# adamgreig/basebandboard

Measured on AMD Instinct MI355X. Metric: awgn_clt_gsamples_per_s, higher is better.
Workload: dtype u32 bit-sliced GF(2) / int8 out

## Files before the change

### basebandboard_amd/csrc/awgn_kernels.hip

```cpp
#include "bbb_common.hpp"
#include "bitslice_util.hpp"
#include "awgn_launch.hpp"
#include "stage_common.hpp"

#include <cstdlib>
#include <mutex>
#include <type_traits>
#include "gen/lutopt256_gen.inc"

namespace bbb {


template <int W32, typename TabPtr>
__device__ __forceinline__ void nibble_matvec_part(TabPtr tab, int nlo, int nhi, const uint32_t (&x)[W32],
                                                   uint32_t (&y)[W32]) {
    constexpr int C = (W32 % 4 == 0) ? 4 : (W32 % 2 == 0 ? 2 : 1);
    constexpr int NC = W32 / C;
    typedef uint32_t chunk_t __attribute__((ext_vector_type(C)));
#pragma unroll
    for (int w = 0; w < W32; w++) {
        uint32_t xw = x[w];
        asm volatile("" : "+v"(xw));
#pragma unroll
        for (int q = 0; q < 8; q += 2) {
// ... 457 lines not shown
        }
        auto load_windows = [&](const unsigned ihalf, uint32_t (&win)[16]) {
#pragma unroll
            for (unsigned e = 0; e < 16; e++) {
                const unsigned j = 8 * (e >> 2) + 4 * ihalf + (e & 3);
                const unsigned long long g = gen_index(wave, lane, j);
                win[e] = 0;
                if (g < G && tx.use_bits) {
                    const uint32_t off = (uint32_t)g * L + r * 16u;
                    const uint32_t rel = (off >> 3) + tx.rel_base;
                    const uint32_t byte = min(rel >> 3, tx.last_word * 4u - 4u);
                    typedef uint32_t __attribute__((aligned(1))) u32_unaligned;
                    win[e] = *reinterpret_cast<const u32_unaligned *>(reinterpret_cast<const char *>(tx.bits) + byte);
                }
            }
        };
        asm volatile("" ::: "memory");
        auto load_z = [&](const unsigned i, uint32_t (&zz)[16]) {
#pragma unroll
            for (int w = 0; w < 4; w++)
#pragma unroll
                for (int t = 0; t < 4; t++) zz[4 * w + t] = Z[((4 * w + t) * 8 + i) * 64 + lane];
        };
        auto round_end = [&](auto full_c, const unsigned i, const uint32_t (&w4)[4], const uint32_t (&zz)[16]) {
            constexpr bool FULL = decltype(full_c)::value;
            uint32_t o[4][4];
#pragma unroll
            for (int w = 0; w < 4; w++) {
                uint32_t z[4] = {zz[4 * w], zz[4 * w + 1], zz[4 * w + 2], zz[4 * w + 3]};
                transpose4x4_bytes(z);
#pragma unroll
                for (int q = 0; q < 4; q++) o[w][q] = z[q];
            }
            u32x4 RA[TX ? 4 : 1], RB[TX ? 4 : 1], RC[TX ? 4 : 1];
            if (TX) {
#pragma unroll
                for (unsigned q = 0; q < 4; q++) {
                    const uint32_t gq = (uint32_t)gen_index(wave, lane, 8 * q + i);
                    const uint32_t rel_q = ((gq * L + r * 16u) >> 3) + tx.rel_base;
                    const uint32_t Q4 = ((w4[q] >> (rel_q & 7u)) & 0x3ffu) << 4;
                    RA[q] = *reinterpret_cast<const u32x4 *>(reinterpret_cast<const char *>(TT) + (Q4 & 0xff0u));
                    RB[q] = *reinterpret_cast<const u32x4 *>(reinterpret_cast<const char *>(TT) + ((Q4 >> 1) & 0xff0u));
                    RC[q] = *reinterpret_cast<const u32x4 *>(reinterpret_cast<const char *>(TT) + ((Q4 >> 2) & 0xff0u));
                }
            }
#pragma unroll
            for (unsigned q = 0; q < 4; q++) {
                const unsigned long long g = gen_index(wave, lane, 8 * q + i);
                const unsigned long long off = g * L + (unsigned long long)r * 16;
                if (!FULL && !(g < G && off < nsamples)) continue;
                if (!TX) {
                    int8_t *dst = (int8_t *)dst_;
                    const u32x4 v = {o[0][q], o[1][q], o[2][q], o[3][q]};
                    if (FULL || off + 16 <= nsamples) {
                        *reinterpret_cast<u32x4 *>(dst + off) = v;
                    } else {
                        const unsigned n = (unsigned)(nsamples - off);
                        for (unsigned e = 0; e < n; e++) dst[off + e] = (int8_t)((o[e >> 2][q] >> (8 * (e & 3))) & 0xff);
                    }
                } else {
                    int16_t *dst = (int16_t *)dst_;
                    const u32x4 A = RA[q], B = RB[q], C = RC[q];
                    const u16x2 nv16 = {(uint16_t)(tx.noise_var * 16), (uint16_t)(tx.noise_var * 16)};
                    uint32_t x[8];
#pragma unroll
                    for (int w = 0; w < 4; w++) {
                        const uint32_t u = o[w][q] ^ 0x80808080u;
                        const uint32_t u01 = __builtin_amdgcn_perm(0u, u, 0x0c010c00u);
                        const uint32_t u23 = __builtin_amdgcn_perm(0u, u, 0x0c030c02u);
                        const int d0 = (2 * w) & 3, d1 = (2 * w + 1) & 3;
                        const uint32_t s01 = w < 2 ? bfi_uniform(selmask[d0], A[d0], B[d0]) : bfi_uniform(selmask[d0], B[d0], C[d0]);
                        const uint32_t s23 = w < 2 ? bfi_uniform(selmask[d1], A[d1], B[d1]) : bfi_uniform(selmask[d1], B[d1], C[d1]);
                        const u16x2 m01 = __builtin_bit_cast(u16x2, u01) * nv16 + __builtin_bit_cast(u16x2, s01);
                        const u16x2 m23 = __builtin_bit_cast(u16x2, u23) * nv16 + __builtin_bit_cast(u16x2, s23);
                        x[2 * w] = __builtin_bit_cast(uint32_t, __builtin_bit_cast(i16x2, m01) >> 4);
                        x[2 * w + 1] = __builtin_bit_cast(uint32_t, __builtin_bit_cast(i16x2, m23) >> 4);
                    }
                    if (FULL || off + 16 <= nsamples) {
                        const u32x4 lo = {x[0], x[1], x[2], x[3]}, hi = {x[4], x[5], x[6], x[7]};
                        reinterpret_cast<u32x4 *>(dst + off)[0] = lo;
                        reinterpret_cast<u32x4 *>(dst + off)[1] = hi;
                    } else {
                        const unsigned n = (unsigned)(nsamples - off);
                        for (unsigned e = 0; e < n; e++) dst[off + e] = (int16_t)((x[e >> 1] >> (16 * (e & 1))) & 0xffff);
                    }
                }
            }
        };
        auto all_iterations = [&](auto full_c) {
            if (TX) {
#pragma unroll 1
                for (unsigned ihalf = 0; ihalf < 2; ihalf++) {
                    uint32_t win[16];
                    load_windows(ihalf, win);
                    uint32_t zc[16], zn[16];
                    load_z(4 * ihalf, zn);
#pragma unroll
                    for (unsigned ii = 0; ii < 4; ii++) {
#pragma unroll
                        for (int e = 0; e < 16; e++) zc[e] = zn[e];
                        if (ii < 3) load_z(4 * ihalf + ii + 1, zn);
                        const uint32_t w4[4] = {win[ii], win[4 + ii], win[8 + ii], win[12 + ii]};
                        round_end(full_c, 4 * ihalf + ii, w4, zc);
                    }
                }
            } else {
                const uint32_t none[4] = {0, 0, 0, 0};
                uint32_t zc[16], zn[16];
                load_z(0, zn);
#pragma unroll 1
                for (unsigned i = 0; i < 8; i++) {
#pragma unroll
                    for (int e = 0; e < 16; e++) zc[e] = zn[e];
                    load_z((i + 1) & 7, zn);
                    round_end(full_c, i, none, zc);
                }
            }
        };
        if (wave_full) all_iterations(std::true_type{});
        else all_iterations(std::false_type{});
    }
}

template <bool SMALL>
__global__ void __launch_bounds__(64) __attribute__((amdgpu_waves_per_eu(1, 1)))
awgn256_planes_kernel(const uint32_t *__restrict planes, u32x4 *__restrict stage, unsigned L, unsigned nlanes
) {
    const unsigned lane = threadIdx.x;
    const unsigned long long wave = blockIdx.x;
    const unsigned long long LG = wave * 64 + lane;
    __builtin_amdgcn_s_setprio(3);
    uint32_t a[256], b[256], pa[256], pb[256], cnt[8];
    if constexpr (SMALL) {
#ifdef BBB_SMALL_THROTTLE
        asm volatile("" ::: BBB_SMALL_THROTTLE);
#endif
        const uint32_t voff = (uint32_t)LG * 4u;
#define BBB_PLANE(p) (*reinterpret_cast<const uint32_t *>(reinterpret_cast<const char *>(planes + (size_t)(p) * nlanes) + (unsigned long long)voff))
#define BBB_PARK(p) { const uint32_t v_ = BBB_PLANE(p); BBB_ACC_WRITE(pa[p], v_); }
        LUTOPT256_FOR_PARKED_HI(BBB_PARK)
#undef BBB_PARK
#pragma unroll
        for (int p = 0; p < 256; p++)
            if (!lutopt256_hi_is_parked(p)) a[p] = BBB_PLANE(p);
#undef BBB_PLANE
    } else {
#pragma unroll
        for (int p = 0; p < 256; p++) b[p] = planes[(size_t)p * nlanes + LG];
        lutopt256_advance(b, a);
#define BBB_PARK(p) BBB_ACC_WRITE(pa[p], a[p]);
        LUTOPT256_FOR_PARKED_HI(BBB_PARK)
#undef BBB_PARK
    }
    u32x4 *out = stage_row(stage, wave, L, lane);
#pragma unroll 1
    for (unsigned t = 0; t < L; t += 2) {
        lutopt256_step_parked_hi(a, pa, b, pb, cnt);
        {
        __builtin_nontemporal_store((u32x4){cnt[0], cnt[1], cnt[2], cnt[3]}, out);
        __builtin_nontemporal_store((u32x4){cnt[4], cnt[5], cnt[6], cnt[7]}, out + kStageHalfVecs);
        }
        lutopt256_step_parked_hi(b, pb, a, pa, cnt);
        {
        __builtin_nontemporal_store((u32x4){cnt[0], cnt[1], cnt[2], cnt[3]}, out + kStageStepVecs);
        __builtin_nontemporal_store((u32x4){cnt[4], cnt[5], cnt[6], cnt[7]}, out + kStageStepVecs + kStageHalfVecs);
        }
        out += 2 * kStageStepVecs;
    }
}

int awgn256_planes_launch(const uint32_t *d_planes, void *stage, unsigned L, unsigned nlanes, hipStream_t st, bool small_footprint) {
    if (L & 1) return fail(BBB_EINVAL, "segment length must be even");
    if (small_footprint)
        hipLaunchKernelGGL(awgn256_planes_kernel<true>, dim3(nlanes / 64), dim3(64), 0, st, d_planes, (u32x4 *)stage, L, nlanes);
    else
        hipLaunchKernelGGL(awgn256_planes_kernel<false>, dim3(nlanes / 64), dim3(64), 0, st, d_planes, (u32x4 *)stage, L, nlanes);
    BBB_HIP(hipGetLastError());
    return BBB_OK;
}

constexpr unsigned kUnplaneRaw = kStageUnitBytes, kUnplaneLds = 3 * kStageUnitBytes, kUnplaneLdsTx = kUnplaneLds + 32 * 1024 + 2 * 2048;

template <bool TXM, bool NOWRAP = false>
__global__ void __launch_bounds__(256, 7)
unplane_kernel(const u32x4 *__restrict stage, char *__restrict dst, unsigned long long win_lo, unsigned long long nbytes_, unsigned L,
               unsigned long long G, StageGeom ge, TxFuse tx) {
    extern __shared__ __attribute__((aligned(16))) uint32_t lds[];
    typedef __attribute__((address_space(3))) void *lds_void_ptr;
    const unsigned tid = threadIdx.x, lane = tid & 63;
    const unsigned wv = (unsigned)__builtin_amdgcn_readfirstlane((int)(tid >> 6));
    if (blockIdx.x * ge.per_block >= ge.nunits) return;
    char *const dstw = dst - win_lo;
    const unsigned long long nbytes = win_lo + nbytes_;
    const unsigned l8 = tid & 7, qs = tid >> 3;
    const unsigned wr0 = l8 * 32 + ((((qs >> 2) ^ (2 * ((l8 >> 1) & 3))) << 2) | (qs & 3));
    const unsigned lq = (tid >> 3) & 7, c2 = tid & 7;
    const unsigned rd0 = (wv * 8 + lq) * 32 + ((c2 ^ (2 * ((lq >> 1) & 3))) << 2);
    uint32_t *const tile = lds + 2 * (kUnplaneRaw / 4);
    uint32_t *const T10 = lds + kUnplaneLds / 4;
    uint32_t *const winb = lds + kUnplaneLds / 4 + 8192;
    if (TXM) {
        uint16_t *const TT = reinterpret_cast<uint16_t *>(tile);
        for (int e = (int)tid; e < 256 * 8; e += 256) {
            const int q = e >> 3, j = e & 7, ph = (int)((tx.c0 + (unsigned)j) & 7u);
            int sum = 0;
#pragma unroll
            for (int idx = 0; idx < 8; idx++) {
                const int c = tx.coeffs[8 * idx + ph];
                sum += ((q >> (7 - idx)) & 1) ? c : -c;
            }
            const int shaped = tx.bit_en ? ((int)((unsigned)sum << 20) >> 20) : 0;
            TT[e] = (uint16_t)((unsigned)((shaped - 128 * tx.noise_var) * (NOWRAP ? 1 : 16)) & 0xffffu);
        }
        __syncthreads();
        for (unsigned p = tid; p < 1024 * 8; p += 256) {
            const unsigned q10 = p >> 3, e = 2 * (p & 7);
            const uint32_t lo = TT[(((q10 >> ((tx.c0 + e) >> 3)) & 0xffu) << 3) + (e & 7)];
            const uint32_t hi = TT[(((q10 >> ((tx.c0 + e + 1) >> 3)) & 0xffu) << 3) + ((e + 1) & 7)];
            T10[p] = lo | (hi << 16);
        }
        __syncthreads();
    }
    auto dma_unit = [&](const StagePos &p, unsigned buf) {
        stage_dma_unit(stage, ge, p, L, lds + buf * (kUnplaneRaw / 4), wv, lane);
        if (TXM) {
            const unsigned step0 = p.rg * kStageUnitSteps;
            const unsigned long long wabs = (unsigned long long)ge.w_lo + p.w;
            const long long so = (long long)((wabs * 2048 + p.q8 * 8) * (unsigned long long)L + step0) - (long long)win_lo;
#pragma unroll
            for (unsigned i = 0; i < 2; i++) {
                const unsigned e = (wv * 2 + i) * 64 + lane, row = e >> 1;
                const long long pu = so + (long long)((unsigned long long)((row >> 3) * 64 + (row & 7)) * L);
                uint32_t word = 0;
                if (pu > -128 && pu < (long long)nbytes_) word = (((uint32_t)(pu >> 3) + tx.rel_base) >> 5) + (e & 1);
                word = word < tx.last_word ? word : tx.last_word;
                __builtin_amdgcn_global_load_lds((const void *)(tx.bits + word), (lds_void_ptr)(uintptr_t)(winb + buf * 512 + (wv * 2 + i) * 64), 4, 0, 0);
            }
        }
    };
    auto wait_vm = [](unsigned n) {
        switch (n) {
#define BBB_W(N) case N: asm volatile("s_waitcnt vmcnt(" #N ")" ::: "memory"); break;
            BBB_W(8) BBB_W(10) BBB_W(16) BBB_W(26)
#undef BBB_W
        default: asm volatile("s_waitcnt vmcnt(0)" ::: "memory"); break;
        }
    };
    constexpr unsigned NDMA = TXM ? 10 : 8, NST = TXM ? 16 : 8;
    StagePos cur;
    const unsigned n_it = stage_block_units(ge, blockIdx.x, &cur);
    StagePos nxt = cur;
    stage_advance(nxt, ge);
    unsigned buf = 0;
    bool fast1 = false;
    dma_unit(cur, 0);
    for (unsigned it = 0; it < n_it; it++, buf ^= 1) {
        const unsigned q8 = cur.q8, step0 = cur.rg * 128;
        const unsigned long long w = (unsigned long long)ge.w_lo + cur.w;
        const bool more1 = it + 1 < n_it;
        if (more1) dma_unit(nxt, buf ^ 1);
        wait_vm((more1 ? NDMA : 0u) + (fast1 ? NST : 0u));
        __builtin_amdgcn_s_barrier();
        {
            uint32_t Z[4][8];
            stage_unpack<TXM>(lds + buf * (kUnplaneRaw / 4), tid, Z);
#pragma unroll
            for (unsigned s = 0; s < 4; s++) planes8_to_bytes(Z[s]);
#pragma unroll
            for (unsigned i = 0; i < 8; i++) {
                uint32_t z[4] = {Z[0][i], Z[1][i], Z[2][i], Z[3][i]};
                transpose4x4_bytes(z);
#pragma unroll
                for (unsigned q = 0; q < 4; q++) tile[wr0 + (8 * q + i) * 256] = z[q];
            }
        }
        asm volatile("s_waitcnt lgkmcnt(0)" ::: "memory");
        __builtin_amdgcn_s_barrier();
        const unsigned inseg = step0 + c2 * 16;
        const unsigned long long g0 = (w * 32 + wv) * 64 + q8 * 8 + lq;
        unsigned long long off = g0 * (unsigned long long)L + inseg;
        const unsigned long long goff = 256ull * L;
        const bool lane_fast = inseg < L && g0 + 7 * 256 < G && off >= win_lo && off + 7 * goff + 16 <= nbytes;
        const bool wave_fast = __all(lane_fast);
        fast1 = wave_fast;
        if (!TXM && inseg < L) {
            if (wave_fast) {
#pragma unroll
                for (unsigned k = 0; k < 8; k++) {
                    const u32x4 v = *reinterpret_cast<const u32x4 *>(&tile[rd0 + k * 1024]);
                    *reinterpret_cast<u32x4 *>(dstw + off) = v;
                    off += goff;
                }
            } else {
                for (unsigned k = 0; k < 8; k++, off += goff) {
                    if (g0 + 256ull * k >= G || off >= nbytes) break;
                    if (off < win_lo) continue;
                    const u32x4 v = *reinterpret_cast<const u32x4 *>(&tile[rd0 + k * 1024]);
                    if (off + 16 <= nbytes) {
                        *reinterpret_cast<u32x4 *>(dstw + off) = v;
                    } else {
                        const unsigned n = (unsigned)(nbytes - off);
                        for (unsigned e = 0; e < n; e++) dstw[off + e] = (char)((v[e >> 2] >> (8 * (e & 3))) & 0xff);
                    }
                }
            }
        }
        if (TXM && inseg < L) {
            int16_t *const dst16 = reinterpret_cast<int16_t *>(dst);
            const u16x2 nv16 = {(uint16_t)(tx.noise_var * (NOWRAP ? 1 : 16)), (uint16_t)(tx.noise_var * (NOWRAP ? 1 : 16))};
            const uint32_t idx_mask = tx.use_bits ? 0x7fe0u : 0u;
            const uint32_t sh = ((((uint32_t)((long long)(off - win_lo) >> 3)) + tx.rel_base - 2u * c2) & 31u) + 2u * c2;
            const uint32_t *const wb0 = winb + buf * 512 + (wv * 8 + lq) * 2;
            auto piece = [&](auto full_c, unsigned k, unsigned long long o) {
                constexpr bool FULL = decltype(full_c)::value;
                typedef uint32_t u32x2 __attribute__((ext_vector_type(2)));
                const u32x2 ww = *reinterpret_cast<const u32x2 *>(wb0 + k * 64);
                const u32x4 v = *reinterpret_cast<const u32x4 *>(&tile[rd0 + k * 1024]);
                const uint32_t wk = (uint32_t)((((unsigned long long)ww[1] << 32) | ww[0]) >> sh);
                const char *const row = reinterpret_cast<const char *>(T10) + ((wk << 5) & idx_mask);
                const u32x4 A = *reinterpret_cast<const u32x4 *>(row);
                const u32x4 B = *reinterpret_cast<const u32x4 *>(row + 16);
                uint32_t x[8];
#pragma unroll
                for (int w4 = 0; w4 < 4; w4++) {
                    const uint32_t u01 = __builtin_amdgcn_perm(0u, v[w4], 0x0c010c00u);
                    const uint32_t u23 = __builtin_amdgcn_perm(0u, v[w4], 0x0c030c02u);
                    const uint32_t s01 = w4 < 2 ? A[2 * w4] : B[2 * w4 - 4], s23 = w4 < 2 ? A[2 * w4 + 1] : B[2 * w4 - 3];
                    const u16x2 m01 = __builtin_bit_cast(u16x2, u01) * nv16 + __builtin_bit_cast(u16x2, s01);
                    const u16x2 m23 = __builtin_bit_cast(u16x2, u23) * nv16 + __builtin_bit_cast(u16x2, s23);
                    if constexpr (NOWRAP) {
                        x[2 * w4] = __builtin_bit_cast(uint32_t, m01);
                        x[2 * w4 + 1] = __builtin_bit_cast(uint32_t, m23);
                    } else {
                        x[2 * w4] = __builtin_bit_cast(uint32_t, __builtin_bit_cast(i16x2, m01) >> 4);
                        x[2 * w4 + 1] = __builtin_bit_cast(uint32_t, __builtin_bit_cast(i16x2, m23) >> 4);
                    }
                }
                int16_t *out = dst16 + (o - win_lo);
                if (FULL || o + 16 <= nbytes) {
                    const u32x4 lo = {x[0], x[1], x[2], x[3]}, hi = {x[4], x[5], x[6], x[7]};
                    reinterpret_cast<u32x4 *>(out)[0] = lo;
                    reinterpret_cast<u32x4 *>(out)[1] = hi;
                } else {
                    const unsigned n = (unsigned)(nbytes - o);
                    for (unsigned e = 0; e < n; e++) out[e] = (int16_t)((x[e >> 1] >> (16 * (e & 1))) & 0xffff);
                }
            };
            if (wave_fast) {
#pragma unroll 1
                for (unsigned k4 = 0; k4 < 8; k4 += 4) {
#pragma unroll
                    for (unsigned k = 0; k < 4; k++) piece(std::true_type{}, k4 + k, off + (k4 + k) * goff);
                }
            } else {
#pragma unroll 1
                for (unsigned k = 0; k < 8; k++) {
                    const unsigned long long o = off + k * goff;
                    if (g0 + 256ull * k >= G || o >= nbytes) break;
                    if (o < win_lo) continue;
                    piece(std::false_type{}, k, o);
                }
            }
        }
        asm volatile("s_waitcnt lgkmcnt(0)" ::: "memory");
        __builtin_amdgcn_s_barrier();
        cur = nxt;
        stage_advance(nxt, ge);
    }
}

static bool unplane_tx_nowrap(const TxFuse &tx) {
    int worst = 0;
    if (tx.bit_en)
        for (int ph = 0; ph < 8; ph++) {
            int sum = 0;
            for (int idx = 0; idx < 8; idx++) sum += tx.coeffs[8 * idx + ph] < 0 ? -(int)tx.coeffs[8 * idx + ph] : (int)tx.coeffs[8 * idx + ph];
            worst = sum > worst ? sum : worst;
        }
    return tx.noise_var >= 0 && worst + 128 * tx.noise_var <= 2047;
}

static int unplane_launch_with(const void *stage, void *dst, uint64_t win_lo, uint64_t nbytes, unsigned L, uint64_t G, unsigned nlanes,
                               const TxFuse *tx, hipStream_t st) {
    if (win_lo & 15) return fail(BBB_EINVAL, "window must start on a 16-byte boundary of the staged stream");
    if (nbytes == 0) return BBB_OK;
    int dev = 0, ncu = 256;
    BBB_HIP(hipGetDevice(&dev));
    BBB_HIP(hipDeviceGetAttribute(&ncu, hipDeviceAttributeMultiprocessorCount, dev));
    StageGeom ge;
    const unsigned blocks = stage_geom(win_lo, nbytes, L, nlanes, (uint64_t)ncu * (uint64_t)env_knob("BBB_UNPLANE_BLOCKS_PER_CU", 1), &ge);
    if (!blocks) return fail(BBB_EINVAL, "staged window too large for one mover launch (2^32 units of 32 KiB)");
    {
        static std::mutex mu;
        static bool attr_set[64] = {false};
        std::lock_guard<std::mutex> g(mu);
        if (dev < 0 || dev >= 64 || !attr_set[dev]) {
            BBB_HIP(hipFuncSetAttribute((const void *)unplane_kernel<false>, hipFuncAttributeMaxDynamicSharedMemorySize, (int)kUnplaneLds));
            BBB_HIP(hipFuncSetAttribute((const void *)unplane_kernel<true>, hipFuncAttributeMaxDynamicSharedMemorySize, (int)kUnplaneLdsTx));
            BBB_HIP(hipFuncSetAttribute((const void *)unplane_kernel<true, true>, hipFuncAttributeMaxDynamicSharedMemorySize, (int)kUnplaneLdsTx));
            if (dev >= 0 && dev < 64) attr_set[dev] = true;
        }
    }
    if (tx && unplane_tx_nowrap(*tx)) {
        hipLaunchKernelGGL((unplane_kernel<true, true>), dim3(blocks), dim3(256), kUnplaneLdsTx, st, (const u32x4 *)stage, (char *)dst,
                           (unsigned long long)win_lo, (unsigned long long)nbytes, L, (unsigned long long)G, ge, *tx);
    } else if (tx) {
        hipLaunchKernelGGL(unplane_kernel<true>, dim3(blocks), dim3(256), kUnplaneLdsTx, st, (const u32x4 *)stage, (char *)dst,
                           (unsigned long long)win_lo, (unsigned long long)nbytes, L, (unsigned long long)G, ge, *tx);
    } else {
        TxFuse none{};
        hipLaunchKernelGGL(unplane_kernel<false>, dim3(blocks), dim3(256), kUnplaneLds, st, (const u32x4 *)stage, (char *)dst,
                           (unsigned long long)win_lo, (unsigned long long)nbytes, L, (unsigned long long)G, ge, none);
    }
    BBB_HIP(hipGetLastError());
    return BBB_OK;
}

int unplane_launch(const void *stage, void *dst, uint64_t win_lo, uint64_t nbytes, unsigned L, uint64_t G, unsigned nlanes, hipStream_t st) {
    return unplane_launch_with(stage, dst, win_lo, nbytes, L, G, nlanes, nullptr, st);
}

int unplane_tx_launch(const void *stage, int16_t *dst, uint64_t win_lo, uint64_t nsamples, unsigned L, uint64_t G, unsigned nlanes,
                      const int16_t *coeffs, const uint32_t *d_bits, uint32_t nwords32, uint32_t rel_base, uint32_t c0, int noise_var, int bit_en,
                      int use_bits, hipStream_t st) {
    const TxFuse tx = make_txfuse(coeffs, d_bits, nwords32, rel_base, c0, noise_var, bit_en, use_bits);
    return unplane_launch_with(stage, dst, win_lo, nsamples, L, G, nlanes, &tx, st);
}

__global__ void __launch_bounds__(256)
widen_i8_i16_kernel(const u32x4 *__restrict src, u32x4 *__restrict dst, unsigned long long n16) {
    const unsigned long long i = (unsigned long long)blockIdx.x * blockDim.x + threadIdx.x;
    if (i >= n16) return;
    const u32x4 v = src[i];
    u32x4 lo, hi;
#pragma unroll
    for (int w = 0; w < 4; w++) {
        const uint32_t x = v[w];
        const uint32_t a = (uint32_t)(uint16_t)(int16_t)(int8_t)(x & 0xff) | ((uint32_t)(uint16_t)(int16_t)(int8_t)((x >> 8) & 0xff) << 16);
        const uint32_t b = (uint32_t)(uint16_t)(int16_t)(int8_t)((x >> 16) & 0xff) | ((uint32_t)(uint16_t)(int16_t)(int8_t)(x >> 24) << 16);
        if (w < 2) { lo[2 * w] = a; lo[2 * w + 1] = b; } else { hi[2 * (w - 2)] = a; hi[2 * (w - 2) + 1] = b; }
    }
    dst[2 * i] = lo;
    dst[2 * i + 1] = hi;
}

int widen_i8_i16_launch(const int8_t *src, int16_t *dst, uint64_t n, hipStream_t st) {
    const unsigned long long n16 = (n + 15) / 16;
    if (!n16) return BBB_OK;
    hipLaunchKernelGGL(widen_i8_i16_kernel, dim3((unsigned)((n16 + 255) / 256)), dim3(256), 0, st,
                       reinterpret_cast<const u32x4 *>(src), reinterpret_cast<u32x4 *>(dst), n16);
    BBB_HIP(hipGetLastError());
    return BBB_OK;
}

template <typename OutT>
__global__ void __launch_bounds__(64)
awgn_generic_kernel(int k, int logk, const uint16_t *__restrict taps, const uint32_t *__restrict row_off,
                    uint32_t *__restrict planes2, OutT *__restrict dst, unsigned long long nsamples, unsigned L,
                    unsigned long long G, unsigned nlanes) {
    const unsigned lane = threadIdx.x;
    const unsigned long long wave = blockIdx.x;
    const unsigned long long LG = wave * 64 + lane;
    uint32_t *cur = planes2, *nxt = planes2 + (size_t)k * nlanes;
    for (unsigned t = 0; t < L; t++) {
        uint32_t c[10];
#pragma unroll
        for (int q = 0; q < 10; q++) c[q] = 0;
        for (int r = 0; r < k; r++) {
            uint32_t acc = 0;
            for (uint32_t e = row_off[r]; e < row_off[r + 1]; e++) acc ^= cur[(size_t)taps[e] * nlanes + LG];
            nxt[(size_t)r * nlanes + LG] = acc;
            uint32_t carry = (__builtin_popcount((unsigned)r) & 1) ? ~acc : acc;
#pragma unroll
            for (int q = 0; q < 10; q++) {
                const uint32_t tcar = c[q] & carry;
                c[q] ^= carry;
                carry = tcar;
            }
        }
        for (unsigned j = 0; j < 32; j++) {
            const unsigned long long g = gen_index(wave, lane, j);
            const unsigned long long off = g * L + t;
            if (g < G && off < nsamples) {
                int T = 0;
#pragma unroll
                for (int q = 0; q < 10; q++) T |= (int)((c[q] >> j) & 1u) << q;
                int v = (T - (k >> 1)) & (k - 1);
                if (v >> (logk - 1)) v -= k;
                dst[off] = (OutT)v;
            }
        }
        uint32_t *sw = cur; cur = nxt; nxt = sw;
    }
}

__global__ void __launch_bounds__(64)
lutopt_words_kernel(int k, const uint16_t *__restrict taps, const uint32_t *__restrict row_off,
                    uint32_t *__restrict planes2, uint32_t *__restrict dst, unsigned long long nstates, unsigned L,
                    unsigned long long G, unsigned nlanes, int msb_first) {
    const unsigned lane = threadIdx.x;
    const unsigned long long wave = blockIdx.x;
    const unsigned long long LG = wave * 64 + lane;
    const unsigned wps = (unsigned)k / 32;
    uint32_t *cur = planes2, *nxt = planes2 + (size_t)k * nlanes;
    for (unsigned t = 0; t < L; t++) {
        for (int r = 0; r < k; r++) {
            uint32_t acc = 0;
            for (uint32_t e = row_off[r]; e < row_off[r + 1]; e++) acc ^= cur[(size_t)taps[e] * nlanes + LG];
            nxt[(size_t)r * nlanes + LG] = acc;
        }
        for (unsigned wq = 0; wq < wps; wq++) {
            uint32_t q[32];
#pragma unroll
            for (int p = 0; p < 32; p++) q[p] = nxt[(size_t)(32 * wq + p) * nlanes + LG];
            transpose32(q);
#pragma unroll
            for (unsigned j = 0; j < 32; j++) {
                const unsigned long long g = gen_index(wave, lane, j);
                const unsigned long long off = g * L + t;
                if (g < G && off < nstates) dst[off * wps + wq] = msb_first ? __builtin_bitreverse32(q[j]) : q[j];
// ... 308 lines not shown
```

### basebandboard_amd/csrc/hist_kernels.hip

```cpp
#include "bbb_common.hpp"
#include "bitslice_util.hpp"
#include "stage_common.hpp"

#include <algorithm>
#include <mutex>

namespace bbb {

typedef uint32_t hist_u32x4 __attribute__((ext_vector_type(4)));

constexpr unsigned kHistLanes = 64;
constexpr unsigned kHistRaw = kStageUnitBytes;
constexpr unsigned kHistTable = 256 * kHistLanes * 4;
constexpr unsigned kHistPlanesLds = kHistTable + 2 * kHistRaw;
constexpr int kHistSampleThreads = 1024;

__device__ __forceinline__ uint32_t hist_fold(const uint32_t *H, unsigned bin) {
    uint32_t sum = 0;
    for (unsigned l = 0; l < kHistLanes; l++) sum += H[bin * kHistLanes + ((l + bin) & (kHistLanes - 1))];
    return sum;
}

__global__ void __launch_bounds__(256, 7)
hist_planes_kernel(const hist_u32x4 *__restrict stage, unsigned long long nsamples, unsigned L, StageGeom ge, uint32_t *__restrict scratch) {
    extern __shared__ __attribute__((aligned(16))) uint32_t lds[];
    typedef __attribute__((address_space(3))) void *lds_void_ptr;
    const unsigned tid = threadIdx.x, lane = tid & 63;
    const unsigned wv = (unsigned)__builtin_amdgcn_readfirstlane((int)(tid >> 6));
    uint32_t *const H = lds;
    uint32_t *const raw0 = lds + kHistTable / 4;
    {
        hist_u32x4 *h4 = reinterpret_cast<hist_u32x4 *>(H);
        for (unsigned i = tid; i < kHistTable / 16; i += 256) h4[i] = hist_u32x4{0u, 0u, 0u, 0u};
    }
    __syncthreads();
    const unsigned l8 = tid & 7, qs = tid >> 3;
    const uint32_t hbase = (uint32_t)(uintptr_t)(lds_void_ptr)H;
    const uint32_t column = lane * 4u;
    StagePos cur;
    const unsigned n_it = stage_block_units(ge, blockIdx.x, &cur);
    StagePos nxt = cur;
    stage_advance(nxt, ge);
    unsigned buf = 0;
    if (n_it) stage_dma_unit(stage, ge, cur, L, raw0, wv, lane);
    for (unsigned it = 0; it < n_it; it++, buf ^= 1) {
        const bool more = it + 1 < n_it;
        if (more) stage_dma_unit(stage, ge, nxt, L, raw0 + (buf ^ 1) * (kHistRaw / 4), wv, lane);
        if (more) asm volatile("s_waitcnt vmcnt(8)" ::: "memory");
        else asm volatile("s_waitcnt vmcnt(0)" ::: "memory");
        __builtin_amdgcn_s_barrier();
        {
            uint32_t Z[4][8];
            stage_unpack<true>(raw0 + buf * (kHistRaw / 4), tid, Z);
#pragma unroll
            for (unsigned s = 0; s < 4; s++) planes8_to_bytes(Z[s]);
            const unsigned step = cur.rg * 128 + 4 * qs;
            const unsigned long long span = 64ull * L;
            const unsigned long long off0 = (((unsigned long long)ge.w_lo + cur.w) * kStageWaveGens + cur.q8 * 8 + l8) * L + step;
#define BBB_HIST_ADD(WORD, Q) \
    asm volatile("ds_add_u32 %0, %1" ::"v"(hbase + __builtin_amdgcn_perm(column, (WORD), 0x0c0c0004u | ((Q) << 8))), "v"(1u) : "memory")
            if (step + 3 < L && off0 + 3 + 31 * span < nsamples) {
#pragma unroll
                for (unsigned s = 0; s < 4; s++) {
#pragma unroll
                    for (unsigned i = 0; i < 8; i++) {
                        BBB_HIST_ADD(Z[s][i], 0u); BBB_HIST_ADD(Z[s][i], 1u); BBB_HIST_ADD(Z[s][i], 2u); BBB_HIST_ADD(Z[s][i], 3u);
                    }
                }
            } else {
#pragma unroll
                for (unsigned s = 0; s < 4; s++) {
                    const unsigned long long o = off0 + s;
                    unsigned nj = 0;
                    if (step + s < L && o < nsamples) {
                        const unsigned long long m = (nsamples - o - 1) / span + 1;
                        nj = m < 32 ? (unsigned)m : 32u;
                    }
#pragma unroll
                    for (unsigned i = 0; i < 8; i++) {
                        if (i < nj) BBB_HIST_ADD(Z[s][i], 0u);
                        if (i + 8 < nj) BBB_HIST_ADD(Z[s][i], 1u);
                        if (i + 16 < nj) BBB_HIST_ADD(Z[s][i], 2u);
                        if (i + 24 < nj) BBB_HIST_ADD(Z[s][i], 3u);
                    }
                }
            }
#undef BBB_HIST_ADD
        }
        asm volatile("s_waitcnt lgkmcnt(0)" ::: "memory");
        __builtin_amdgcn_s_barrier();
        cur = nxt;
        stage_advance(nxt, ge);
    }
    __syncthreads();
    scratch[(size_t)blockIdx.x * 256 + tid] = hist_fold(H, tid);
}

template <typename T>
__global__ void __launch_bounds__(kHistSampleThreads)
hist_samples_kernel(const T *__restrict x, unsigned long long nsamples, unsigned nbins, uint32_t *__restrict scratch) {
    extern __shared__ __attribute__((aligned(16))) uint32_t lds[];
    uint32_t *const H = lds;
    for (unsigned i = threadIdx.x; i < nbins * kHistLanes; i += kHistSampleThreads) H[i] = 0u;
    __syncthreads();
    constexpr unsigned PER = 16 / sizeof(T);
    const unsigned lane = threadIdx.x & 63, half = nbins >> 1, mask = nbins - 1;
    const unsigned long long ngroups = nsamples / PER;
    const hist_u32x4 *xv = reinterpret_cast<const hist_u32x4 *>(x);
    const unsigned long long stride = (unsigned long long)gridDim.x * kHistSampleThreads;
    for (unsigned long long g = (unsigned long long)blockIdx.x * kHistSampleThreads + threadIdx.x; g < ngroups; g += stride) {
        const hist_u32x4 v = xv[g];
#pragma unroll
        for (unsigned e = 0; e < PER; e++) {
            int s;
            if (sizeof(T) == 1) s = (int)(int8_t)((v[e >> 2] >> (8 * (e & 3))) & 0xffu);
            else s = (int)(int16_t)((v[e >> 1] >> (16 * (e & 1))) & 0xffffu);
            atomicAdd(&H[(((unsigned)s + half) & mask) * kHistLanes + lane], 1u);
        }
    }
    if (blockIdx.x == 0) {
        const unsigned long long i = ngroups * PER + threadIdx.x;
        if (threadIdx.x < PER && i < nsamples) atomicAdd(&H[(((unsigned)(int)x[i] + half) & mask) * kHistLanes + lane], 1u);
    }
    __syncthreads();
    for (unsigned bin = threadIdx.x; bin < nbins; bin += kHistSampleThreads) scratch[(size_t)blockIdx.x * nbins + bin] = hist_fold(H, bin);
}

__global__ void __launch_bounds__(256)
hist_reduce_kernel(const uint32_t *__restrict scratch, unsigned used, unsigned nbins, unsigned long long *__restrict hist) {
    const unsigned t = blockIdx.x * 256 + threadIdx.x;
    if (t >= nbins) return;
    unsigned long long sum = 0;
    for (unsigned b = 0; b < used; b++) sum += scratch[(size_t)b * nbins + t];
    hist[t] += sum;
}

int hist_grid_blocks() {
    int dev = 0, cus = 0;
    BBB_HIP(hipGetDevice(&dev));
    BBB_HIP(hipDeviceGetAttribute(&cus, hipDeviceAttributeMultiprocessorCount, dev));
    return std::max(cus, 1);
}

static int hist_lds_attributes() {
    static std::mutex mu;
    static bool attr_set[64] = {false};
    int dev = 0;
    BBB_HIP(hipGetDevice(&dev));
    std::lock_guard<std::mutex> g(mu);
    if (dev < 0 || dev >= 64 || !attr_set[dev]) {
        const int most = (int)(kHistMaxBins * kHistLanes * 4);
        BBB_HIP(hipFuncSetAttribute((const void *)hist_planes_kernel, hipFuncAttributeMaxDynamicSharedMemorySize, (int)kHistPlanesLds));
        BBB_HIP(hipFuncSetAttribute((const void *)hist_samples_kernel<int8_t>, hipFuncAttributeMaxDynamicSharedMemorySize, most));
        BBB_HIP(hipFuncSetAttribute((const void *)hist_samples_kernel<int16_t>, hipFuncAttributeMaxDynamicSharedMemorySize, most));
        if (dev >= 0 && dev < 64) attr_set[dev] = true;
    }
    return BBB_OK;
}

int hist_planes_launch(const void *stage, uint64_t nsamples, unsigned L, unsigned nlanes, uint32_t *scratch, int blocks, unsigned *used,
                       hipStream_t st) {
    if (nsamples == 0 || nsamples > (1ull << 31)) return fail(BBB_EINVAL, "a histogram launch counts 1 .. 2^31 samples");
    if (L == 0 || blocks < 1) return fail(BBB_EINVAL, "bad histogram launch");
    StageGeom ge;
    const unsigned nb = stage_geom(0, nsamples, L, nlanes, (uint64_t)blocks, &ge);
    if (!nb) return fail(BBB_EINVAL, "staged range out of the histogram mover's reach");
    int rc = hist_lds_attributes();
    if (rc) return rc;
    hipLaunchKernelGGL(hist_planes_kernel, dim3(nb), dim3(256), kHistPlanesLds, st, (const hist_u32x4 *)stage, (unsigned long long)nsamples, L, ge,
                       scratch);
    BBB_HIP(hipGetLastError());
    *used = nb;
    return BBB_OK;
}

int hist_samples_launch(const void *samples, int elem, uint64_t nsamples, unsigned nbins, uint32_t *scratch, int blocks, unsigned *used,
                        hipStream_t st) {
    if (nsamples == 0 || nsamples > (1ull << 31)) return fail(BBB_EINVAL, "a histogram launch counts 1 .. 2^31 samples");
    if (nbins < 2 || nbins > kHistMaxBins || (nbins & (nbins - 1)) || blocks < 1 || ((uintptr_t)samples & 15) || (elem != 1 && elem != 2))
        return fail(BBB_EINVAL, "bad histogram launch");
    int rc = hist_lds_attributes();
    if (rc) return rc;
    const uint64_t want = (nsamples + (uint64_t)kHistSampleThreads * 256 - 1) / ((uint64_t)kHistSampleThreads * 256);
    const unsigned nb = (unsigned)std::max<uint64_t>(1, std::min<uint64_t>(want, (uint64_t)blocks));
    const size_t smem = (size_t)nbins * kHistLanes * 4;
    if (elem == 1)
        hipLaunchKernelGGL(hist_samples_kernel<int8_t>, dim3(nb), dim3(kHistSampleThreads), smem, st, (const int8_t *)samples,
                           (unsigned long long)nsamples, nbins, scratch);
    else
        hipLaunchKernelGGL(hist_samples_kernel<int16_t>, dim3(nb), dim3(kHistSampleThreads), smem, st, (const int16_t *)samples,
                           (unsigned long long)nsamples, nbins, scratch);
    BBB_HIP(hipGetLastError());
    *used = nb;
    return BBB_OK;
}

int hist_reduce_launch(const uint32_t *scratch, unsigned used, unsigned nbins, uint64_t *hist, hipStream_t st) {
    hipLaunchKernelGGL(hist_reduce_kernel, dim3((nbins + 255) / 256), dim3(256), 0, st, scratch, used, nbins,
                       reinterpret_cast<unsigned long long *>(hist));
    BBB_HIP(hipGetLastError());
    return BBB_OK;
}

}
```

### basebandboard_amd/csrc/stage_common.hpp

```cpp
#pragma once

#include <algorithm>
#include <cstddef>
#include <cstdint>

namespace bbb {

constexpr unsigned kStageLaneBytes = 16;
constexpr unsigned kStageHalfBytes = 64 * kStageLaneBytes;
constexpr unsigned kStageStepBytes = 2 * kStageHalfBytes;
constexpr unsigned kStageHalfVecs = kStageHalfBytes / 16, kStageStepVecs = kStageStepBytes / 16;
constexpr unsigned kStageWaveGens = 64 * 32;
constexpr unsigned kStageUnitLanes = 8, kStageUnitSteps = 128;
constexpr unsigned kStageUnitBytes = kStageUnitLanes * kStageUnitSteps * 2 * kStageLaneBytes;

inline size_t stage_words(unsigned nlanes, uint64_t L) { return (size_t)(nlanes / 64) * (size_t)L * (kStageStepBytes / 4); }

struct StageGeom {
    unsigned w_lo, ngroups, nunits;
    unsigned per_block;
};

inline unsigned stage_geom(uint64_t win_lo, uint64_t n, unsigned L, unsigned nlanes, uint64_t blocks_wanted, StageGeom *ge) {
    const uint64_t seg = (uint64_t)L * kStageWaveGens;
    const uint64_t w_lo = win_lo / seg;
    const uint64_t w_hi = std::min<uint64_t>((win_lo + n + seg - 1) / seg, nlanes / 64);
    ge->w_lo = (unsigned)w_lo;
    ge->ngroups = (L + kStageUnitSteps - 1) / kStageUnitSteps;
    const uint64_t nunits = w_hi > w_lo ? (w_hi - w_lo) * ge->ngroups * (64 / kStageUnitLanes) : 0;
    if (nunits == 0 || nunits >> 32) return 0;
    ge->nunits = (unsigned)nunits;
    const uint64_t want = std::max<uint64_t>(1, std::min<uint64_t>(blocks_wanted, nunits));
    ge->per_block = (unsigned)((nunits + want - 1) / want);
    return (unsigned)((nunits + ge->per_block - 1) / ge->per_block);
}

#ifdef __HIPCC__

typedef uint32_t stage_u32x4 __attribute__((ext_vector_type(4)));

__device__ __forceinline__ stage_u32x4 *stage_row(stage_u32x4 *stage, unsigned long long wave, unsigned L, unsigned lane) {
    return stage + (wave * L) * kStageStepVecs + lane;
}

struct StagePos { unsigned q8, rg, w; };

__device__ __forceinline__ void stage_advance(StagePos &p, const StageGeom &ge) {
    if (++p.rg == ge.ngroups) {
        p.rg = 0;
        if (++p.q8 == 64 / kStageUnitLanes) { p.q8 = 0; p.w++; }
    }
}

__device__ __forceinline__ unsigned stage_block_units(const StageGeom &ge, unsigned block, StagePos *first) {
    const unsigned u0 = block * ge.per_block;
    first->rg = u0 % ge.ngroups;
    first->q8 = (u0 / ge.ngroups) & 7;
    first->w = (u0 / ge.ngroups) >> 3;
    return u0 >= ge.nunits ? 0u : (ge.nunits - u0 < ge.per_block ? ge.nunits - u0 : ge.per_block);
}

__device__ __forceinline__ const char *stage_unit_src(const void *stage, unsigned long long wabs, unsigned L, unsigned step0, unsigned q8) {
    return reinterpret_cast<const char *>(stage) + ((wabs * L + step0) * kStageStepVecs + q8 * kStageUnitLanes) * 16;
}

__device__ __forceinline__ void stage_dma_unit(const void *stage, const StageGeom &ge, const StagePos &p, unsigned L, uint32_t *raw, unsigned wv,
                                               unsigned lane) {
    typedef __attribute__((address_space(3))) void *lds_void_ptr;
    const unsigned step0 = p.rg * kStageUnitSteps;
    const char *const sb = stage_unit_src(stage, (unsigned long long)ge.w_lo + p.w, L, step0, p.q8);
    uint32_t *const rawb = raw + wv * 8 * 256;
    if (step0 + kStageUnitSteps <= L) {
        const char *const pl = sb + wv * kStageStepBytes + (lane & 7) * 16 + (lane >> 3) * (4 * kStageStepBytes);
#pragma unroll
        for (unsigned k = 0; k < 8; k++)
            __builtin_amdgcn_global_load_lds((const void *)(pl + ((k & 3) * 32 * kStageStepBytes + (k >> 2) * kStageHalfBytes)),
                                             (lds_void_ptr)(uintptr_t)(rawb + k * 256), 16, 0, 0);
    } else {
        const unsigned last = L - 1 - step0;
#pragma unroll
        for (unsigned k = 0; k < 8; k++) {
            unsigned st = 4 * ((k & 3) * 8 + (lane >> 3)) + wv;
            st = st < last ? st : last;
            __builtin_amdgcn_global_load_lds((const void *)(sb + (size_t)st * kStageStepBytes + (k >> 2) * kStageHalfBytes + (lane & 7) * 16),
                                             (lds_void_ptr)(uintptr_t)(rawb + k * 256), 16, 0, 0);
        }
    }
}

template <bool COMPLEMENT7>
__device__ __forceinline__ void stage_unpack(const uint32_t *raw_image, unsigned tid, uint32_t (&Z)[4][8]) {
    const uint32_t *raw = raw_image + ((tid >> 3) * 8 + (tid & 7)) * 4;
#pragma unroll
    for (unsigned s = 0; s < 4; s++) {
        const stage_u32x4 lo = *reinterpret_cast<const stage_u32x4 *>(raw + (2 * s) * 1024);
        const stage_u32x4 hi = *reinterpret_cast<const stage_u32x4 *>(raw + (2 * s + 1) * 1024);
        Z[s][0] = lo[0]; Z[s][1] = lo[1]; Z[s][2] = lo[2]; Z[s][3] = lo[3];
        Z[s][4] = hi[0]; Z[s][5] = hi[1]; Z[s][6] = hi[2]; Z[s][7] = COMPLEMENT7 ? ~hi[3] : hi[3];
    }
}

#endif

}
```

Before: 965.3.

## Skip storing high count planes when zero, using per-step flag bitmaps

Splits each stage step record into a 16-byte low part, an 8-byte mid part and an 8-byte tail part (planes 6-7). The tail is written only when some lane has nonzero bits there, which a wave ballot decides, and a per-step flag bitmap records this. Consumer kernels prefetch the flags and load the tail only when it was written, otherwise rebuilding planes 6/7 from plane 5. The aim is to cut stage write and read traffic, at the cost of extra flag loads and stores, buffer-descriptor setup, and more complex unpacking.

After: 994.3, median of 6. 1.03x the previous value.

```diff
diff --git a/basebandboard_amd/csrc/awgn_kernels.hip b/basebandboard_amd/csrc/awgn_kernels.hip
--- a/basebandboard_amd/csrc/awgn_kernels.hip
+++ b/basebandboard_amd/csrc/awgn_kernels.hip
@@ -633,20 +633,24 @@
         LUTOPT256_FOR_PARKED_HI(BBB_PARK)
 #undef BBB_PARK
     }
-    u32x4 *out = stage_row(stage, wave, L, lane);
+    u32x4 *rec = stage_row(stage, wave, L, 0);
+    uint32_t flags = 0;
 #pragma unroll 1
-    for (unsigned t = 0; t < L; t += 2) {
-        lutopt256_step_parked_hi(a, pa, b, pb, cnt);
-        {
-        __builtin_nontemporal_store((u32x4){cnt[0], cnt[1], cnt[2], cnt[3]}, out);
-        __builtin_nontemporal_store((u32x4){cnt[4], cnt[5], cnt[6], cnt[7]}, out + kStageHalfVecs);
-        }
-        lutopt256_step_parked_hi(b, pb, a, pa, cnt);
-        {
-        __builtin_nontemporal_store((u32x4){cnt[0], cnt[1], cnt[2], cnt[3]}, out + kStageStepVecs);
-        __builtin_nontemporal_store((u32x4){cnt[4], cnt[5], cnt[6], cnt[7]}, out + kStageStepVecs + kStageHalfVecs);
-        }
-        out += 2 * kStageStepVecs;
+    for (unsigned t32 = 0; t32 < L; t32 += 32) {
+        const unsigned tend = L - t32 < 32 ? L : t32 + 32;
+#pragma unroll 1
+        for (unsigned t = t32; t < tend; t += 2) {
+            lutopt256_step_parked_hi(a, pa, b, pb, cnt);
+            {
+            stage_store_step(rec, lane, cnt, t, flags);
+            }
+            lutopt256_step_parked_hi(b, pb, a, pa, cnt);
+            {
+            stage_store_step(rec + kStageStepVecs, lane, cnt, t + 1, flags);
+            }
+            rec += 2 * kStageStepVecs;
+        }
+        stage_store_flags(stage, nlanes, L, wave, tend - 1, flags);
     }
 }
 
@@ -660,7 +664,7 @@
     return BBB_OK;
 }
 
-constexpr unsigned kUnplaneRaw = kStageUnitBytes, kUnplaneLds = 3 * kStageUnitBytes, kUnplaneLdsTx = kUnplaneLds + 32 * 1024 + 2 * 2048;
+constexpr unsigned kUnplaneRaw = kStageRawBytes, kUnplaneLds = 3 * kStageRawBytes, kUnplaneLdsTx = kUnplaneLds + 32 * 1024 + 2 * 2048;
 
 template <bool TXM, bool NOWRAP = false>
 __global__ void __launch_bounds__(256, 7)
@@ -702,8 +706,8 @@
         }
         __syncthreads();
     }
-    auto dma_unit = [&](const StagePos &p, unsigned buf) {
-        stage_dma_unit(stage, ge, p, L, lds + buf * (kUnplaneRaw / 4), wv, lane);
+    auto dma_unit = [&](const StagePos &p, const StageFlags f, unsigned buf) {
+        stage_dma_unit(stage, ge, p, f, L, lds + buf * (kUnplaneRaw / 4), wv, lane);
         if (TXM) {
             const unsigned step0 = p.rg * kStageUnitSteps;
             const unsigned long long wabs = (unsigned long long)ge.w_lo + p.w;
@@ -728,23 +732,23 @@
         }
     };
     constexpr unsigned NDMA = TXM ? 10 : 8, NST = TXM ? 16 : 8;
-    StagePos cur;
-    const unsigned n_it = stage_block_units(ge, blockIdx.x, &cur);
-    StagePos nxt = cur;
-    stage_advance(nxt, ge);
+    StageWalk wk;
+    const unsigned n_it = stage_walk_begin(wk, stage, ge, blockIdx.x, L);
     unsigned buf = 0;
     bool fast1 = false;
-    dma_unit(cur, 0);
+    dma_unit(wk.cur, wk.fcur, 0);
     for (unsigned it = 0; it < n_it; it++, buf ^= 1) {
+        const StagePos cur = wk.cur;
         const unsigned q8 = cur.q8, step0 = cur.rg * 128;
         const unsigned long long w = (unsigned long long)ge.w_lo + cur.w;
         const bool more1 = it + 1 < n_it;
-        if (more1) dma_unit(nxt, buf ^ 1);
+        if (more1) dma_unit(wk.nxt, wk.fnxt, buf ^ 1);
+        stage_walk_prefetch(wk, stage, ge, L, it, n_it);
         wait_vm((more1 ? NDMA : 0u) + (fast1 ? NST : 0u));
         __builtin_amdgcn_s_barrier();
         {
             uint32_t Z[4][8];
-            stage_unpack<TXM>(lds + buf * (kUnplaneRaw / 4), tid, Z);
+            stage_unpack<TXM>(lds + buf * (kUnplaneRaw / 4), wk.fcur, tid, Z);
 #pragma unroll
             for (unsigned s = 0; s < 4; s++) planes8_to_bytes(Z[s]);
 #pragma unroll
@@ -845,8 +849,7 @@
         }
         asm volatile("s_waitcnt lgkmcnt(0)" ::: "memory");
         __builtin_amdgcn_s_barrier();
-        cur = nxt;
-        stage_advance(nxt, ge);
+        stage_walk_step(wk, ge);
     }
 }
 
diff --git a/basebandboard_amd/csrc/hist_kernels.hip b/basebandboard_amd/csrc/hist_kernels.hip
--- a/basebandboard_amd/csrc/hist_kernels.hip
+++ b/basebandboard_amd/csrc/hist_kernels.hip
@@ -10,7 +10,7 @@
 typedef uint32_t hist_u32x4 __attribute__((ext_vector_type(4)));
 
 constexpr unsigned kHistLanes = 64;
-constexpr unsigned kHistRaw = kStageUnitBytes;
+constexpr unsigned kHistRaw = kStageRawBytes;
 constexpr unsigned kHistTable = 256 * kHistLanes * 4;
 constexpr unsigned kHistPlanesLds = kHistTable + 2 * kHistRaw;
 constexpr int kHistSampleThreads = 1024;
@@ -37,21 +37,21 @@
     const unsigned l8 = tid & 7, qs = tid >> 3;
     const uint32_t hbase = (uint32_t)(uintptr_t)(lds_void_ptr)H;
     const uint32_t column = lane * 4u;
-    StagePos cur;
-    const unsigned n_it = stage_block_units(ge, blockIdx.x, &cur);
-    StagePos nxt = cur;
-    stage_advance(nxt, ge);
+    StageWalk wk;
+    const unsigned n_it = stage_walk_begin(wk, stage, ge, blockIdx.x, L);
     unsigned buf = 0;
-    if (n_it) stage_dma_unit(stage, ge, cur, L, raw0, wv, lane);
+    if (n_it) stage_dma_unit(stage, ge, wk.cur, wk.fcur, L, raw0, wv, lane);
     for (unsigned it = 0; it < n_it; it++, buf ^= 1) {
+        const StagePos cur = wk.cur;
         const bool more = it + 1 < n_it;
-        if (more) stage_dma_unit(stage, ge, nxt, L, raw0 + (buf ^ 1) * (kHistRaw / 4), wv, lane);
+        if (more) stage_dma_unit(stage, ge, wk.nxt, wk.fnxt, L, raw0 + (buf ^ 1) * (kHistRaw / 4), wv, lane);
+        stage_walk_prefetch(wk, stage, ge, L, it, n_it);
         if (more) asm volatile("s_waitcnt vmcnt(8)" ::: "memory");
         else asm volatile("s_waitcnt vmcnt(0)" ::: "memory");
         __builtin_amdgcn_s_barrier();
         {
             uint32_t Z[4][8];
-            stage_unpack<true>(raw0 + buf * (kHistRaw / 4), tid, Z);
+            stage_unpack<true>(raw0 + buf * (kHistRaw / 4), wk.fcur, tid, Z);
 #pragma unroll
             for (unsigned s = 0; s < 4; s++) planes8_to_bytes(Z[s]);
             const unsigned step = cur.rg * 128 + 4 * qs;
@@ -89,8 +89,7 @@
         }
         asm volatile("s_waitcnt lgkmcnt(0)" ::: "memory");
         __builtin_amdgcn_s_barrier();
-        cur = nxt;
-        stage_advance(nxt, ge);
+        stage_walk_step(wk, ge);
     }
     __syncthreads();
     scratch[(size_t)blockIdx.x * 256 + tid] = hist_fold(H, tid);
diff --git a/basebandboard_amd/csrc/stage_common.hpp b/basebandboard_amd/csrc/stage_common.hpp
--- a/basebandboard_amd/csrc/stage_common.hpp
+++ b/basebandboard_amd/csrc/stage_common.hpp
@@ -7,18 +7,31 @@
 namespace bbb {
 
 constexpr unsigned kStageLaneBytes = 16;
-constexpr unsigned kStageHalfBytes = 64 * kStageLaneBytes;
-constexpr unsigned kStageStepBytes = 2 * kStageHalfBytes;
-constexpr unsigned kStageHalfVecs = kStageHalfBytes / 16, kStageStepVecs = kStageStepBytes / 16;
+constexpr unsigned kStagePairBytes = 8;
+constexpr unsigned kStageStepBytes = 2048;
+constexpr unsigned kStageRowB = 64 * kStageLaneBytes, kStageRowC = kStageRowB + 64 * kStagePairBytes;
+constexpr unsigned kStageStepVecs = kStageStepBytes / 16;
 constexpr unsigned kStageWaveGens = 64 * 32;
 constexpr unsigned kStageUnitLanes = 8, kStageUnitSteps = 128;
-constexpr unsigned kStageUnitBytes = kStageUnitLanes * kStageUnitSteps * 2 * kStageLaneBytes;
+constexpr unsigned kStageRawA = 0, kStageRawB = kStageUnitLanes * kStageUnitSteps * kStageLaneBytes;
+constexpr unsigned kStageRawC = kStageRawB + kStageUnitLanes * kStageUnitSteps * kStagePairBytes;
+constexpr unsigned kStageRawBytes = kStageRawC + kStageUnitLanes * kStageUnitSteps * kStagePairBytes;
 
-inline size_t stage_words(unsigned nlanes, uint64_t L) { return (size_t)(nlanes / 64) * (size_t)L * (kStageStepBytes / 4); }
+inline constexpr unsigned stage_flag_words(uint64_t L) { return (unsigned)((L + kStageUnitSteps - 1) / kStageUnitSteps) * (kStageUnitSteps / 32); }
+
+inline size_t stage_words(unsigned nlanes, uint64_t L) {
+    return (size_t)(nlanes / 64) * ((size_t)L * (kStageStepBytes / 4) + stage_flag_words(L));
+}
+
+inline constexpr size_t stage_flag_word(unsigned nlanes, uint64_t L, uint64_t wave, uint64_t step) {
+    return (size_t)(nlanes / 64) * (size_t)L * kStageStepBytes + ((size_t)wave * stage_flag_words(L) + (size_t)(step >> 5)) * 4;
+}
+inline constexpr uint32_t stage_flag_bit(uint64_t step) { return 1u << (step & 31); }
 
 struct StageGeom {
     unsigned w_lo, ngroups, nunits;
     unsigned per_block;
+    unsigned nlanes;
 };
 
 inline unsigned stage_geom(uint64_t win_lo, uint64_t n, unsigned L, unsigned nlanes, uint64_t blocks_wanted, StageGeom *ge) {
@@ -26,6 +39,7 @@
     const uint64_t w_lo = win_lo / seg;
     const uint64_t w_hi = std::min<uint64_t>((win_lo + n + seg - 1) / seg, nlanes / 64);
     ge->w_lo = (unsigned)w_lo;
+    ge->nlanes = nlanes;
     ge->ngroups = (L + kStageUnitSteps - 1) / kStageUnitSteps;
     const uint64_t nunits = w_hi > w_lo ? (w_hi - w_lo) * ge->ngroups * (64 / kStageUnitLanes) : 0;
     if (nunits == 0 || nunits >> 32) return 0;
@@ -39,8 +53,28 @@
 
 typedef uint32_t stage_u32x4 __attribute__((ext_vector_type(4)));
 
+typedef uint32_t stage_u32x2 __attribute__((ext_vector_type(2)));
+
 __device__ __forceinline__ stage_u32x4 *stage_row(stage_u32x4 *stage, unsigned long long wave, unsigned L, unsigned lane) {
     return stage + (wave * L) * kStageStepVecs + lane;
+}
+
+__device__ __forceinline__ void stage_store_step(stage_u32x4 *rec, unsigned lane, const uint32_t (&cnt)[8], unsigned step, uint32_t &flags) {
+    constexpr int kRaw32 = 0x00020000, kNonTemporal = 2;
+    const uint32_t off16 = lane * kStageLaneBytes, off8 = lane * kStagePairBytes;
+    const uint32_t tail = __builtin_amdgcn_bitop3_b32(cnt[5], cnt[6], cnt[7], 0x7e);
+    const bool any = __builtin_amdgcn_ballot_w64(tail != 0u) != 0ull;
+    const __amdgpu_buffer_rsrc_t rs = __builtin_amdgcn_make_buffer_rsrc(rec, 0, (int)kStageStepBytes, kRaw32);
+    const __amdgpu_buffer_rsrc_t rs_tail = __builtin_amdgcn_make_buffer_rsrc(rec, 0, any ? (int)kStageStepBytes : 0, kRaw32);
+    __builtin_amdgcn_raw_buffer_store_b128((stage_u32x4){cnt[0], cnt[1], cnt[2], cnt[3]}, rs, (int)off16, 0, kNonTemporal);
+    __builtin_amdgcn_raw_buffer_store_b64((stage_u32x2){cnt[4], cnt[5]}, rs, (int)off8, (int)kStageRowB, kNonTemporal);
+    __builtin_amdgcn_raw_buffer_store_b64((stage_u32x2){cnt[6], cnt[7]}, rs_tail, (int)off8, (int)kStageRowC, kNonTemporal);
+    flags |= any ? stage_flag_bit(step) : 0u;
+}
+
+__device__ __forceinline__ void stage_store_flags(void *stage, unsigned nlanes, unsigned L, unsigned long long wave, unsigned step, uint32_t &flags) {
+    *reinterpret_cast<uint32_t *>(reinterpret_cast<char *>(stage) + stage_flag_word(nlanes, L, wave, step)) = flags;
+    flags = 0u;
 }
 
 struct StagePos { unsigned q8, rg, w; };
@@ -64,39 +98,92 @@
     return reinterpret_cast<const char *>(stage) + ((wabs * L + step0) * kStageStepVecs + q8 * kStageUnitLanes) * 16;
 }
 
-__device__ __forceinline__ void stage_dma_unit(const void *stage, const StageGeom &ge, const StagePos &p, unsigned L, uint32_t *raw, unsigned wv,
-                                               unsigned lane) {
+typedef stage_u32x4 StageFlags;
+
+__device__ __forceinline__ StageFlags stage_unit_flags(const void *stage, const StageGeom &ge, const StagePos &p, unsigned L) {
+    typedef const __attribute__((address_space(4))) stage_u32x4 *const_u32x4_ptr;
+    const char *const fw = reinterpret_cast<const char *>(stage) + stage_flag_word(ge.nlanes, L, (unsigned long long)ge.w_lo + p.w, p.rg * kStageUnitSteps);
+    return *(const_u32x4_ptr)(uintptr_t)fw;
+}
+
+struct StageWalk {
+    StagePos cur, nxt, nn;
+    StageFlags fcur, fnxt, fnn;
+};
+
+__device__ __forceinline__ unsigned stage_walk_begin(StageWalk &wk, const void *stage, const StageGeom &ge, unsigned block, unsigned L) {
+    const unsigned n = stage_block_units(ge, block, &wk.cur);
+    wk.nxt = wk.cur;
+    stage_advance(wk.nxt, ge);
+    wk.nn = wk.nxt;
+    stage_advance(wk.nn, ge);
+    wk.fcur = wk.fnxt = wk.fnn = StageFlags{0u, 0u, 0u, 0u};
+    if (n > 0) wk.fcur = stage_unit_flags(stage, ge, wk.cur, L);
+    if (n > 1) wk.fnxt = stage_unit_flags(stage, ge, wk.nxt, L);
+    return n;
+}
+
+__device__ __forceinline__ void stage_walk_prefetch(StageWalk &wk, const void *stage, const StageGeom &ge, unsigned L, unsigned it, unsigned n) {
+    if (it + 2 < n) wk.fnn = stage_unit_flags(stage, ge, wk.nn, L);
+}
+
+__device__ __forceinline__ void stage_walk_step(StageWalk &wk, const StageGeom &ge) {
+    wk.cur = wk.nxt; wk.fcur = wk.fnxt;
+    wk.nxt = wk.nn; wk.fnxt = wk.fnn;
+    stage_advance(wk.nn, ge);
+}
+
+__device__ __forceinline__ void stage_dma_unit(const void *stage, const StageGeom &ge, const StagePos &p, const StageFlags f, unsigned L, uint32_t *raw,
+                                               unsigned wv, unsigned lane) {
     typedef __attribute__((address_space(3))) void *lds_void_ptr;
     const unsigned step0 = p.rg * kStageUnitSteps;
     const char *const sb = stage_unit_src(stage, (unsigned long long)ge.w_lo + p.w, L, step0, p.q8);
-    uint32_t *const rawb = raw + wv * 8 * 256;
-    if (step0 + kStageUnitSteps <= L) {
-        const char *const pl = sb + wv * kStageStepBytes + (lane & 7) * 16 + (lane >> 3) * (4 * kStageStepBytes);
+    const char *const sb8 = sb - p.q8 * (kStageUnitLanes * kStageLaneBytes) + kStageRowB + p.q8 * (kStageUnitLanes * kStagePairBytes);
+    uint32_t *const rawa = raw + kStageRawA / 4 + wv * 1024, *const rawb = raw + kStageRawB / 4 + wv * 512, *const rawc = raw + kStageRawC / 4 + wv * 512;
+    const bool whole = step0 + kStageUnitSteps <= L;
+    const unsigned last = whole ? kStageUnitSteps - 1 : L - 1 - step0;
 #pragma unroll
-        for (unsigned k = 0; k < 8; k++)
-            __builtin_amdgcn_global_load_lds((const void *)(pl + ((k & 3) * 32 * kStageStepBytes + (k >> 2) * kStageHalfBytes)),
-                                             (lds_void_ptr)(uintptr_t)(rawb + k * 256), 16, 0, 0);
-    } else {
-        const unsigned last = L - 1 - step0;
+    for (unsigned k = 0; k < 4; k++) {
+        unsigned st = 4 * (k * 8 + (lane >> 3)) + wv;
+        st = st < last ? st : last;
+        __builtin_amdgcn_global_load_lds((const void *)(sb + (size_t)st * kStageStepBytes + (lane & 7) * 16), (lds_void_ptr)(uintptr_t)(rawa + k * 256), 16, 0,
+                                         0);
+    }
 #pragma unroll
-        for (unsigned k = 0; k < 8; k++) {
-            unsigned st = 4 * ((k & 3) * 8 + (lane >> 3)) + wv;
-            st = st < last ? st : last;
-            __builtin_amdgcn_global_load_lds((const void *)(sb + (size_t)st * kStageStepBytes + (k >> 2) * kStageHalfBytes + (lane & 7) * 16),
-                                             (lds_void_ptr)(uintptr_t)(rawb + k * 256), 16, 0, 0);
-        }
+    for (unsigned k = 0; k < 2; k++) {
+        unsigned st = 4 * (k * 16 + (lane >> 2)) + wv;
+        st = st < last ? st : last;
+        __builtin_amdgcn_global_load_lds((const void *)(sb8 + (size_t)st * kStageStepBytes + (lane & 3) * 16), (lds_void_ptr)(uintptr_t)(rawb + k * 256), 16, 0,
+                                         0);
+    }
+#pragma unroll
+    for (unsigned k = 0; k < 2; k++) {
+        unsigned st = 4 * (k * 16 + (lane >> 2)) + wv;
+        st = st < last ? st : last;
+        const uint32_t word = (lane & 32u) ? f[2 * k + 1] : f[2 * k];
+        const bool tail = (word >> (4 * ((lane >> 2) & 7u) + wv)) & 1u;
+        const char *const src = tail ? sb8 + (size_t)st * kStageStepBytes + (kStageRowC - kStageRowB) + (lane & 3) * 16 : sb8;
+        __builtin_amdgcn_global_load_lds((const void *)src, (lds_void_ptr)(uintptr_t)(rawc + k * 256), 16, 0, 0);
     }
 }
 
 template <bool COMPLEMENT7>
-__device__ __forceinline__ void stage_unpack(const uint32_t *raw_image, unsigned tid, uint32_t (&Z)[4][8]) {
-    const uint32_t *raw = raw_image + ((tid >> 3) * 8 + (tid & 7)) * 4;
+__device__ __forceinline__ void stage_unpack(const uint32_t *raw_image, const StageFlags f, unsigned tid, uint32_t (&Z)[4][8]) {
+    const unsigned at = (tid >> 3) * 8 + (tid & 7);
+    const uint32_t *const rawa = raw_image + kStageRawA / 4 + at * 4, *const rawb = raw_image + kStageRawB / 4 + at * 2,
+                   *const rawc = raw_image + kStageRawC / 4 + at * 2;
+    const unsigned wv = (unsigned)__builtin_amdgcn_readfirstlane((int)(tid >> 6));
+    const uint32_t word = wv & 2u ? (wv & 1u ? f[3] : f[2]) : (wv & 1u ? f[1] : f[0]);
+    const uint32_t mine = word >> (4 * ((tid >> 3) & 7u));
 #pragma unroll
     for (unsigned s = 0; s < 4; s++) {
-        const stage_u32x4 lo = *reinterpret_cast<const stage_u32x4 *>(raw + (2 * s) * 1024);
-        const stage_u32x4 hi = *reinterpret_cast<const stage_u32x4 *>(raw + (2 * s + 1) * 1024);
+        const stage_u32x4 lo = *reinterpret_cast<const stage_u32x4 *>(rawa + s * 1024);
+        const stage_u32x2 mid = *reinterpret_cast<const stage_u32x2 *>(rawb + s * 512);
+        const stage_u32x2 hi = *reinterpret_cast<const stage_u32x2 *>(rawc + s * 512);
+        const bool tail = (mine >> s) & 1u;
+        const uint32_t p7 = tail ? hi[1] : mid[1];
         Z[s][0] = lo[0]; Z[s][1] = lo[1]; Z[s][2] = lo[2]; Z[s][3] = lo[3];
-        Z[s][4] = hi[0]; Z[s][5] = hi[1]; Z[s][6] = hi[2]; Z[s][7] = COMPLEMENT7 ? ~hi[3] : hi[3];
+        Z[s][4] = mid[0]; Z[s][5] = mid[1]; Z[s][6] = tail ? hi[0] : mid[1]; Z[s][7] = COMPLEMENT7 ? ~p7 : p7;
     }
 }
 
```
